# rom1504/clip-retrieval

Hardware: AMD Instinct MI355X
Metric: images/sec embedded (ViT-L/14 bs=256; each sample = image + caption through both towers) (higher is better)
Workload: dtype bf16

## Files before the change

clip-retrieval_amd/csrc/clip_kernels.h:

```cpp
#pragma once
#include <hip/hip_runtime.h>
#include <stdint.h>

namespace clipx {

typedef __bf16 bf16;

enum GemmEpilogue {
  EPI_BIAS_BF16 = 0,
  EPI_BIAS_QGELU_BF16 = 1,
  EPI_BIAS_GELU_BF16 = 2,
  EPI_BIAS_RESID_F32 = 3,
  EPI_TABLE_F32 = 4,
  EPI_RAW_F32 = 5,
  EPI_BIAS_RESID_H16 = 6,
  EPI_BIAS_F16 = 7
};

struct GemmArgs {
  const bf16* A;
  const bf16* W;
  const float* bias;
  void* out;
  const float* table;
  int T;
  int M, N, K;
  int epi;
  int variant;
  int n_cu;
  int row0;
  const float* rowscale;
  bf16* out16;
  float* splitk_ws;
  size_t splitk_ws_bytes;
  int tail_m0, tail_nb;
  int f16;
  float stats_eps;
  int* range_flag;
};

int gemm256_bulk_mtiles(int M, int N, int n_cu);
int gemm256_tail_blocks(int N, int K, int n_cu);

hipError_t launch_gemm(const GemmArgs& g, hipStream_t st);

hipError_t launch_layernorm(const float* x, const float* gamma, const float* beta, void* y, int out_kind, int M,
                            int d, float eps, hipStream_t st, bf16* y16 = nullptr);

hipError_t launch_rowstats(const void* x16, float* rstd, int M, int d, float eps, hipStream_t st, int f16 = 0, int* range_flag = nullptr,
                           int canonical = 0);

hipError_t launch_fold_layernorm(const float* W, const float* gamma, const float* beta, const float* bias, bf16* Wf, float* cf,
                                 int N, int K, hipStream_t st, int f16 = 0);
hipError_t launch_fill_f32(float* p, float v, int64_t n, hipStream_t st);

hipError_t launch_im2col(const void* pixels, int fmt, int B, int S, int P, int Kp, const float* mean,
                         const float* stdv, bf16* out, hipStream_t st);

hipError_t launch_attention(const bf16* qkv, bf16* out, int B, int T, int H, int dh, int causal, hipStream_t st, int q_blocks = 0,
                            const int* offs = nullptr, const int* lens = nullptr);

hipError_t launch_text_embed(const int32_t* ids, const float* tok_emb, const float* pos_emb, float* x, int B, int T,
                             int d, int vocab, hipStream_t st, void* x16 = nullptr, int x16_f16 = 0, const int* rowmap = nullptr,
                             int nrows = 0);

hipError_t launch_gather_pooled(const bf16* att, const void* x16, const int32_t* ids_or_null, bf16* attc, void* xc, int B, int T,
                                int d, hipStream_t st, const int* rows_or_null = nullptr);
hipError_t launch_tail(const void* x, const int32_t* ids_or_null, const float* gamma, const float* beta,
                       const bf16* proj, uint16_t* out_f16, float* out_f32_or_null, float* scratch, int B, int T, int d,
                       int E, float eps, hipStream_t st, int x_f16 = 0, int* range_flag = nullptr);

hipError_t launch_f32_to_bf16(const float* in, bf16* out, int64_t n, hipStream_t st);
hipError_t launch_pad_rows_bf16(const float* in, bf16* out, int rows, int k, int kp, hipStream_t st);

}
```

clip-retrieval_amd/csrc/clip_kernels.hip:

```cpp

#include <hip/hip_runtime.h>
#include <stdint.h>
#include <stdlib.h>
#include <math.h>
#include "clip_kernels.h"
#include "gemm_common.h"

namespace clipx {

constexpr int G_TM = 128, G_TN = 128, G_BK = 64;
constexpr int G_STAGE_BYTES = (G_TM + G_TN) * G_BK * 2;
constexpr int G_GROUP_M = 8;

template <int EPI, bool GLDS, bool DEEP = false, bool F16 = false>
__global__ __launch_bounds__(256, (DEEP && !CLIPX_MFMA16) ? 1 : 2) void gemm_bf16_kernel(const bf16* __restrict__ A, const bf16* __restrict__ W,
                                                          const float* __restrict__ bias, void* __restrict__ outp,
                                                          const float* __restrict__ table, int T, int M, int N,
                                                          int K, int row0, const float* __restrict__ rowscale,
                                                          bf16* __restrict__ out16, int kz) {
  extern __shared__ __attribute__((aligned(16))) unsigned char smem[];
  const int tid = threadIdx.x;
  const int lane = tid & 63, w = tid >> 6;
  const int wn = w & 1, wm = w >> 1;
  const int hb = lane >> 5, l31 = lane & 31;
// ... 375 lines not shown
}

static hipError_t launch_gemm128(const GemmArgs& g, hipStream_t st) {
  const bool small_off = (size_t)g.M * g.K * 2 < ((size_t)1 << 32) && (size_t)g.N * g.K * 2 < ((size_t)1 << 32);
  const int S = (g.variant == 1 && small_off) ? splitk_factor(g) : 1;
  if (S > 1) {
    switch (g.epi) {
      case EPI_BIAS_BF16: return launch_splitk_epi<EPI_BIAS_BF16>(g, S, st);
      case EPI_BIAS_F16: return launch_splitk_epi<EPI_BIAS_F16>(g, S, st);
      case EPI_BIAS_QGELU_BF16: return launch_splitk_epi<EPI_BIAS_QGELU_BF16>(g, S, st);
      case EPI_BIAS_GELU_BF16: return launch_splitk_epi<EPI_BIAS_GELU_BF16>(g, S, st);
      case EPI_BIAS_RESID_F32: return launch_splitk_epi<EPI_BIAS_RESID_F32>(g, S, st);
      case EPI_BIAS_RESID_H16: return launch_splitk_epi<EPI_BIAS_RESID_H16>(g, S, st);
      default: break;
    }
  }
  if (g.f16) {
    switch (g.epi) {
      case EPI_BIAS_BF16: return launch_gemm_epi<EPI_BIAS_BF16, true>(g, st);
      case EPI_BIAS_F16: return launch_gemm_epi<EPI_BIAS_F16, true>(g, st);
      case EPI_BIAS_QGELU_BF16: return launch_gemm_epi<EPI_BIAS_QGELU_BF16, true>(g, st);
      case EPI_BIAS_GELU_BF16: return launch_gemm_epi<EPI_BIAS_GELU_BF16, true>(g, st);
      default: return hipErrorInvalidValue;
    }
  }
  switch (g.epi) {
    case EPI_BIAS_BF16: return launch_gemm_epi<EPI_BIAS_BF16>(g, st);
    case EPI_BIAS_F16: return launch_gemm_epi<EPI_BIAS_F16>(g, st);
    case EPI_BIAS_QGELU_BF16: return launch_gemm_epi<EPI_BIAS_QGELU_BF16>(g, st);
    case EPI_BIAS_GELU_BF16: return launch_gemm_epi<EPI_BIAS_GELU_BF16>(g, st);
    case EPI_BIAS_RESID_F32: return launch_gemm_epi<EPI_BIAS_RESID_F32>(g, st);
    case EPI_BIAS_RESID_H16: return launch_gemm_epi<EPI_BIAS_RESID_H16>(g, st);
    case EPI_TABLE_F32: return launch_gemm_epi<EPI_TABLE_F32>(g, st);
    default: return hipErrorInvalidValue;
  }
}

int gemm256_bulk_mtiles(int M, int N, int n_cu) {
  const int mt = M / 256, nt = N / 256;
  if (mt <= 0 || nt <= 0) return 0;
  const int cu = (n_cu > 0 ? n_cu : 256) & ~7;
  int best = mt;
  double best_cost = 1e30;
  for (int peel = 0; peel <= 8 && peel < mt; ++peel) {
    const int bulk = mt - peel;
    const int rounds = (bulk * nt + cu - 1) / cu;
    const double rest = (double)(peel * 4 * nt) / (2.0 * cu);
    const double cost = rounds + (peel ? 0.25 * (rest > 1.0 ? rest : 1.0) / 0.6 : 0.0);
    if (cost < best_cost - 1e-9) { best_cost = cost; best = bulk; }
  }
  return best;
}

int gemm256_tail_blocks(int N, int K, int n_cu) {
  int grid = (n_cu > 0 ? n_cu : 256) & ~7;
  if (grid < 8) grid = 8;
  if (N % 32 || K % 128 || (size_t)32 * K * 2 >= ((size_t)1 << 31)) return 0;
  const int cb = N / 32;
  for (int nb = 1; nb <= 4; ++nb)
    if (cb % nb == 0 && 8 * (cb / nb) <= grid) return nb;
  return 0;
}

hipError_t launch_gemm(const GemmArgs& g0, hipStream_t st) {
  GemmArgs g = g0;
  if (g.M <= 0 || g.N % G_TN != 0 || g.K % G_BK != 0 || g.K <= 0) return hipErrorInvalidValue;
  const bool out16 = g.epi == EPI_BIAS_BF16 || g.epi == EPI_BIAS_QGELU_BF16 || g.epi == EPI_BIAS_GELU_BF16 || g.epi == EPI_BIAS_F16;
  if (out16 && !g.rowscale) return hipErrorInvalidValue;
  if (g.f16 && !out16) return hipErrorInvalidValue;
  if (g.stats_eps > 0.f) {
    if (!g.f16 || !out16) return hipErrorInvalidValue;
    int fused_rows = 0;
    if (g.variant == 6 && g.N % 256 == 0 && g.K % 128 == 0 && g.M >= 256) {
      const int bulk = gemm256_bulk_mtiles(g.M, g.N, g.n_cu);
      const int cu = (g.n_cu > 0 ? g.n_cu : 256);
      GemmArgs b = g;
      b.M = bulk * 256;
      if (bulk > 0 && (int64_t)bulk * (g.N / 256) >= cu / 2 && gemm256w4_fuses_stats(b)) fused_rows = b.M;
    }
    if (fused_rows < g.M) {
      hipError_t e = launch_rowstats(reinterpret_cast<const char*>(g.A) + (size_t)fused_rows * g.K * 2, const_cast<float*>(g.rowscale) + fused_rows,
                                     g.M - fused_rows, g.K, g.stats_eps, st, 1, g.range_flag, 1);
      if (e != hipSuccess) return e;
    }
    if (fused_rows == 0) g.stats_eps = 0.f;
  }
  if (g.variant >= 2 && g.N % 256 == 0 && g.K % 128 == 0 && g.M >= 256) {
    const int bulk = gemm256_bulk_mtiles(g.M, g.N, g.n_cu);
    const int cu = (g.n_cu > 0 ? g.n_cu : 256);
    if (bulk > 0 && (int64_t)bulk * (g.N / 256) >= cu / 2) {
      GemmArgs b = g;
      b.M = bulk * 256;
      b.tail_m0 = b.tail_nb = 0;
      if (g.M - b.M == 256 && (g.variant == 3 || g.variant == 6) && g.row0 == 0) {
        b.tail_nb = gemm256_tail_blocks(g.N, g.K, g.n_cu);
        b.tail_m0 = b.M;
      }
      const bool tail_inside = b.tail_nb > 0;
      hipError_t e = (g.variant == 6 && gemm256w4_supports(b)) ? launch_gemm256w4(b, g.n_cu, st) : launch_gemm256sp(b, g.n_cu, st);
      if (e != hipSuccess) return e;
      if (b.M == g.M || tail_inside) return hipSuccess;
      GemmArgs r = g;
      r.variant = 1;
      r.stats_eps = 0.f;
      r.splitk_ws = nullptr;
      r.A = g.A + (size_t)b.M * g.K;
      r.M = g.M - b.M;
      const size_t esz = (g.epi == EPI_BIAS_RESID_F32 || g.epi == EPI_TABLE_F32) ? 4 : 2;
      r.out = reinterpret_cast<char*>(g.out) + (size_t)b.M * g.N * esz;
      r.row0 = g.row0 + b.M;
      if (g.rowscale) r.rowscale = g.rowscale + b.M;
      if (g.out16) r.out16 = g.out16 + (size_t)b.M * g.N;
      return launch_gemm128(r, st);
    }
  }
  GemmArgs r = g;
  if (r.variant >= 2) r.variant = 1;
  r.stats_eps = 0.f;
  return launch_gemm128(r, st);
}

template <int NV, int OUT>
__global__ __launch_bounds__(256) void layernorm_kernel(const float* __restrict__ x, const float* __restrict__ gamma,
                                                       const float* __restrict__ beta, void* __restrict__ y, int M,
                                                       float eps, bf16* __restrict__ y16) {
  constexpr int d = NV * 256;
  const int lane = threadIdx.x & 63;
  const int row = blockIdx.x * 4 + (threadIdx.x >> 6);
  if (row >= M) return;
  const float4* xr = reinterpret_cast<const float4*>(x + (size_t)row * d);
  float4 v[NV];
  float s = 0.f;
#pragma unroll
  for (int e = 0; e < NV; ++e) {
    v[e] = xr[lane + 64 * e];
    s += (v[e].x + v[e].y) + (v[e].z + v[e].w);
  }
  for (int o = 32; o > 0; o >>= 1) s += __shfl_xor(s, o);
  const float mean = s * (1.f / d);
  float q = 0.f;
#pragma unroll
  for (int e = 0; e < NV; ++e) {
    const float a = v[e].x - mean, b = v[e].y - mean, c = v[e].z - mean, dd = v[e].w - mean;
    q += (a * a + b * b) + (c * c + dd * dd);
  }
  for (int o = 32; o > 0; o >>= 1) q += __shfl_xor(q, o);
  const float rstd = 1.f / sqrtf(q * (1.f / d) + eps);
#pragma unroll
  for (int e = 0; e < NV; ++e) {
    const int c4 = lane + 64 * e;
    const float4 g4 = reinterpret_cast<const float4*>(gamma)[c4];
    const float4 b4 = reinterpret_cast<const float4*>(beta)[c4];
    float4 o;
    o.x = (v[e].x - mean) * rstd * g4.x + b4.x;
    o.y = (v[e].y - mean) * rstd * g4.y + b4.y;
    o.z = (v[e].z - mean) * rstd * g4.z + b4.z;
    o.w = (v[e].w - mean) * rstd * g4.w + b4.w;
    if (OUT == 1) {
      bf16x4 ob;
      ob[0] = (bf16)o.x; ob[1] = (bf16)o.y; ob[2] = (bf16)o.z; ob[3] = (bf16)o.w;
      reinterpret_cast<bf16x4*>(reinterpret_cast<bf16*>(y) + (size_t)row * d)[c4] = ob;
    } else if (OUT == 2) {
      f16x4 oh;
      oh[0] = (_Float16)o.x; oh[1] = (_Float16)o.y; oh[2] = (_Float16)o.z; oh[3] = (_Float16)o.w;
      reinterpret_cast<f16x4*>(reinterpret_cast<_Float16*>(y) + (size_t)row * d)[c4] = oh;
    } else {
      reinterpret_cast<float4*>(reinterpret_cast<float*>(y) + (size_t)row * d)[c4] = o;
      if (y16) {
// ... 1265 lines not shown
```

clip-retrieval_amd/csrc/clipx_api.hip:

```cpp

#include <hip/hip_runtime.h>
#include <stdint.h>
#include <stdlib.h>
#include <string.h>
#include <algorithm>
#include <map>
#include <mutex>
#include <tuple>
#include <string>
#include <vector>

#include "../../include/clipx.h"
#include "clip_kernels.h"

using namespace clipx;

static thread_local std::string g_err;
static int fail(int code, const std::string& msg) {
  g_err = msg;
  return code;
}
#define HIPCHK(expr)                                                                      \
  do {                                                                                    \
    hipError_t _e = (expr);                                                               \
// ... 159 lines not shown
}

static int create_impl(clipx_handle* h, const float* blob, size_t blob_floats) {
  const clipx_model_desc& d = h->desc;
  const int g = d.image_size / d.patch_size;
  Tower& V = h->vis;
  Tower& X = h->txt;
  V.width = d.v_width; V.layers = d.v_layers; V.heads = d.v_heads; V.mlp = d.v_mlp; V.T = g * g + 1;
  X.width = d.t_width; X.layers = d.t_layers; X.heads = d.t_heads; X.mlp = d.t_mlp; X.T = d.ctx_len;
  h->PP3 = 3 * d.patch_size * d.patch_size;
  h->Kp = (h->PP3 + 63) / 64 * 64;
  const size_t E = d.embed_dim;

  HIPCHK(hipStreamCreateWithFlags(&h->stream, hipStreamNonBlocking));
  HIPCHK(hipStreamCreateWithFlags(&h->copy_stream, hipStreamNonBlocking));
  HIPCHK(hipMalloc((void**)&h->blob_dev, blob_floats * sizeof(float)));
  HIPCHK(hipMemcpy(h->blob_dev, blob, blob_floats * sizeof(float), hipMemcpyHostToDevice));

  int r;
  float* p = h->blob_dev;
  const float* conv32 = p; p += (size_t)V.width * h->PP3;
  const float* cls = p; p += V.width;
  const float* vpos = p; p += (size_t)V.T * V.width;
  h->ln_pre_w = p; p += V.width;
  h->ln_pre_b = p; p += V.width;
  if ((r = dev_alloc(h, (void**)&h->conv_w, (size_t)V.width * h->Kp * sizeof(bf16)))) return r;
  HIPCHK(launch_pad_rows_bf16(conv32, h->conv_w, V.width, h->PP3, h->Kp, h->stream));
  if ((r = dev_alloc(h, (void**)&h->clspos, (size_t)V.T * V.width * sizeof(float)))) return r;
  HIPCHK(hipMemcpyAsync(h->clspos, vpos, (size_t)V.T * V.width * sizeof(float), hipMemcpyDeviceToDevice, h->stream));
  {
    const size_t off_cls = (size_t)(cls - h->blob_dev), off_pos = (size_t)(vpos - h->blob_dev);
    std::vector<float> row0(V.width);
    for (int i = 0; i < V.width; ++i) row0[i] = blob[off_cls + i] + blob[off_pos + i];
    HIPCHK(hipStreamSynchronize(h->stream));
    HIPCHK(hipMemcpy(h->clspos, row0.data(), V.width * sizeof(float), hipMemcpyHostToDevice));
  }
  if ((r = carve_layers(h, V, p))) return r;
  V.lnf_w = p; p += V.width;
  V.lnf_b = p; p += V.width;
  const float* vproj32 = p; p += E * V.width;
  if ((r = dev_alloc(h, (void**)&V.proj, E * V.width * sizeof(bf16)))) return r;
  HIPCHK(launch_f32_to_bf16(vproj32, V.proj, (int64_t)(E * V.width), h->stream));
  h->tok_emb = p; p += (size_t)d.vocab * X.width;
  h->txt_pos = p; p += (size_t)X.T * X.width;
  if ((r = carve_layers(h, X, p))) return r;
  X.lnf_w = p; p += X.width;
  X.lnf_b = p; p += X.width;
  const float* tproj32 = p; p += E * X.width;
  if ((r = dev_alloc(h, (void**)&X.proj, E * X.width * sizeof(bf16)))) return r;
  HIPCHK(launch_f32_to_bf16(tproj32, X.proj, (int64_t)(E * X.width), h->stream));
  if ((size_t)(p - h->blob_dev) != blob_floats) return fail(CLIPX_E_ARG, "internal: blob carve does not match clipx_blob_floats");

  const size_t Bm = h->max_batch;
  const size_t rowsV = Bm * V.T, rowsX = Bm * X.T;
  const size_t nx = std::max(rowsV * V.width, rowsX * X.width);
  const size_t nqkv = std::max(rowsV * 3 * V.width, rowsX * 3 * X.width);
  const size_t nh = std::max(rowsV * V.mlp, rowsX * X.mlp);
  if ((r = dev_alloc(h, (void**)&h->x, rowsV * V.width * sizeof(float)))) return r;
  if ((r = dev_alloc(h, (void**)&h->xn, nx * sizeof(bf16)))) return r;
  if ((r = dev_alloc(h, (void**)&h->rstd, std::max(rowsV, rowsX) * sizeof(float)))) return r;
  if ((r = dev_alloc(h, (void**)&h->qkv, nqkv * sizeof(bf16)))) return r;
  if ((r = dev_alloc(h, (void**)&h->att, nx * sizeof(bf16)))) return r;
  if ((r = dev_alloc(h, (void**)&h->hbuf, nh * sizeof(bf16)))) return r;
  if ((r = dev_alloc(h, (void**)&h->patches, rowsV * h->Kp * sizeof(bf16)))) return r;
  h->splitk_ws_bytes = (size_t)32 << 20;
  if ((r = dev_alloc(h, (void**)&h->splitk_ws, h->splitk_ws_bytes))) return r;

  h->in_slot_bytes = std::max((size_t)Bm * 3 * d.image_size * d.image_size * sizeof(float), (size_t)Bm * d.ctx_len * sizeof(int32_t));
  h->out_slot_bytes = Bm * E * sizeof(uint16_t);
  for (int s = 0; s < clipx_handle::NSLOT; ++s) {
    HIPCHK(hipHostMalloc(&h->pin_in[s], h->in_slot_bytes, hipHostMallocDefault));
    HIPCHK(hipHostMalloc(&h->pin_out[s], h->out_slot_bytes * 3, hipHostMallocDefault));
    if ((r = dev_alloc(h, &h->dev_in[s], h->in_slot_bytes))) return r;
    if ((r = dev_alloc(h, (void**)&h->dev_out[s], h->out_slot_bytes))) return r;
    if ((r = dev_alloc(h, (void**)&h->dev_out32[s], h->out_slot_bytes * 2))) return r;
    HIPCHK(hipEventCreateWithFlags(&h->ev_copied[s], hipEventDisableTiming));
    HIPCHK(hipEventCreateWithFlags(&h->ev_done[s], hipEventDisableTiming));
  }
  HIPCHK(hipEventCreateWithFlags(&h->ev_ws, hipEventDisableTiming));
  if ((r = dev_alloc(h, (void**)&h->range_flags, (clipx_handle::NSLOT + 1) * sizeof(int)))) return r;
  HIPCHK(hipMemsetAsync(h->range_flags, 0, (clipx_handle::NSLOT + 1) * sizeof(int), h->stream));
  HIPCHK(hipHostMalloc((void**)&h->range_host, (clipx_handle::NSLOT + 1) * sizeof(int), hipHostMallocDefault));
  memset(h->range_host, 0, (clipx_handle::NSLOT + 1) * sizeof(int));
  h->cur_flag = h->range_flags + clipx_handle::NSLOT;
  {
    const size_t rg_ints = (size_t)Bm * (X.T + 3);
    for (int i = 0; i < clipx_handle::RG_SLOTS; ++i) {
      HIPCHK(hipHostMalloc((void**)&h->rg_host[i], rg_ints * sizeof(int), hipHostMallocDefault));
      if ((r = dev_alloc(h, (void**)&h->rg_dev[i], rg_ints * sizeof(int)))) return r;
      HIPCHK(hipEventCreateWithFlags(&h->rg_ev[i], hipEventDisableTiming));
    }
    HIPCHK(hipHostMalloc((void**)&h->rg_ids_host, (size_t)Bm * X.T * sizeof(int32_t), hipHostMallocDefault));
  }
  HIPCHK(hipStreamSynchronize(h->stream));
  return 0;
}

extern "C" int clipx_create(const clipx_model_desc* desc, const float* blob, size_t blob_floats, int device,
                            clipx_handle** out) {
  if (!desc || !blob || !out) return fail(CLIPX_E_ARG, "null argument");
  *out = nullptr;
  int r = check_desc(desc);
  if (r) return r;
  if (blob_floats != clipx_blob_floats(desc)) return fail(CLIPX_E_ARG, "weight blob has the wrong number of floats for this model description");
  int ndev = 0;
  HIPCHK(hipGetDeviceCount(&ndev));
  if (device < 0 || device >= ndev) return fail(CLIPX_E_ARG, "no such HIP device");
  HIPCHK(hipSetDevice(device));
  hipDeviceProp_t prop;
  HIPCHK(hipGetDeviceProperties(&prop, device));
  if (std::string(prop.gcnArchName).find("gfx950") == std::string::npos)
    return fail(CLIPX_E_UNSUPPORTED, std::string("kernels are built for gfx950 only, device is ") + prop.gcnArchName);
  clipx_handle* h = new clipx_handle();
  h->desc = *desc;
  h->device = device;
  const char* mb = getenv("CLIPX_MAX_BATCH");
  if (mb && atoi(mb) > 0) h->max_batch = atoi(mb);
  const char* hc = getenv("CLIPX_HOST_CHUNK");
  if (hc && atoi(hc) > 0) h->host_chunk = atoi(hc);
  h->host_chunk = std::min(h->host_chunk, h->max_batch);
  const char* gv = getenv("CLIPX_GEMM_VARIANT");
  if (gv) h->gemm_variant = std::min(6, std::max(0, atoi(gv)));
  const char* lf = getenv("CLIPX_LN_FUSED");
  if (lf) h->ln_fused = lf[0] == '1';
  const char* rgt = getenv("CLIPX_RAGGED_TEXT");
  if (rgt && rgt[0] == '0') h->ragged_text = false;
  const char* fl = getenv("CLIPX_FULL_LAST_BLOCK");
  if (fl && atoi(fl) > 0) h->pool_last_block = false;
  h->n_cu = prop.multiProcessorCount > 0 ? prop.multiProcessorCount : 256;
  r = create_impl(h, blob, blob_floats);
  if (r) {
    std::string keep = g_err;
    clipx_destroy(h);
    g_err = keep;
    return r;
  }
  *out = h;
  return CLIPX_OK;
}
// ... 22 lines not shown
    if (h->rg_ev[i]) (void)hipEventDestroy(h->rg_ev[i]);
  }
  if (h->rg_ids_host) (void)hipHostFree(h->rg_ids_host);
  if (h->range_host) (void)hipHostFree(h->range_host);
  if (h->stream) (void)hipStreamDestroy(h->stream);
  if (h->copy_stream) (void)hipStreamDestroy(h->copy_stream);
  delete h;
}

extern "C" int clipx_set_option(clipx_handle* h, int option, int value) {
  if (!h) return fail(CLIPX_E_ARG, "handle is null");
  std::lock_guard<std::mutex> lk(h->mu);
  switch (option) {
    case CLIPX_OPT_RAGGED_TEXT: h->ragged_text = value != 0; return CLIPX_OK;
    case CLIPX_OPT_POOL_LAST_BLOCK: h->pool_last_block = value != 0; return CLIPX_OK;
    default: return fail(CLIPX_E_ARG, "unknown option");
  }
}
extern "C" int clipx_get_option(const clipx_handle* h, int option) {
  if (!h) return -1;
  switch (option) {
    case CLIPX_OPT_RAGGED_TEXT: return h->ragged_text ? 1 : 0;
    case CLIPX_OPT_POOL_LAST_BLOCK: return h->pool_last_block ? 1 : 0;
    default: return -1;
  }
}
extern "C" int clipx_max_batch(const clipx_handle* h) { return h ? h->max_batch : 0; }
extern "C" int clipx_graphs_cached(const clipx_handle* h) { return h ? (int)h->graphs.size() : 0; }
extern "C" int clipx_embed_dim(const clipx_handle* h) { return h ? h->desc.embed_dim : 0; }

struct ProfScope {
  clipx_handle* h;
  hipStream_t st;
  hipEvent_t a = nullptr, b = nullptr;
  int kind;
  double flops;
  ProfScope(clipx_handle* h_, hipStream_t st_, int kind_, double flops_) : h(h_), st(st_), kind(kind_), flops(flops_) {
    if (h->prof & (1 << kind)) {
      (void)hipEventCreate(&a);
      (void)hipEventCreate(&b);
      (void)hipEventRecord(a, st);
    }
  }
  ~ProfScope() {
    if (a && b) {
      (void)hipEventRecord(b, st);
      h->prof_events.push_back({a, b, kind, flops});
    }
  }
};

static int run_gemm(clipx_handle* h, hipStream_t st, const bf16* A, const bf16* W, const float* bias, void* out,
                    const float* table, int T, int M, int N, int K, int epi, const float* rowscale = nullptr, bool f16 = false,
                    float stats_eps = 0.f) {
  GemmArgs g{};
  g.A = A; g.W = W; g.bias = bias; g.out = out; g.table = table; g.T = T;
  g.M = M; g.N = N; g.K = K; g.epi = epi; g.variant = h->gemm_variant; g.n_cu = h->n_cu; g.row0 = 0;
  g.rowscale = rowscale; g.out16 = nullptr; g.f16 = f16 ? 1 : 0;
  g.stats_eps = stats_eps; g.range_flag = stats_eps > 0.f ? h->cur_flag : nullptr;
  if (h->single_query) { g.splitk_ws = h->splitk_ws; g.splitk_ws_bytes = h->splitk_ws_bytes; }
  ProfScope ps(h, st, 0, 2.0 * M * (double)N * K);
  HIPCHK(launch_gemm(g, st));
  return 0;
}

static const void* pooled_rows(const clipx_handle* h, int B, int width) {
  return reinterpret_cast<const char*>(h->x) + (((size_t)B * width * sizeof(bf16) + 255) & ~(size_t)255);
}

struct Ragged {
  int M;
  const int* offs;
  const int* lens;
  const int* rowmap;
  const int* poolrows;
  double att_flops;
};

static int run_layers(clipx_handle* h, hipStream_t st, const Tower& t, int B, int causal, const int32_t* ids, bool* pooled,
                      const Ragged* rg = nullptr) {
  const int M = rg ? rg->M : B * t.T, w = t.width;
  const float eps = h->desc.ln_eps;
  const int act = h->desc.act == CLIPX_ACT_QUICK_GELU ? EPI_BIAS_QGELU_BF16 : EPI_BIAS_GELU_BF16;
  for (int l = 0; l < t.layers; ++l) {
    const LayerW& L = t.L[l];
    int r;
    if (!h->ln_fused) { ProfScope ps(h, st, 2, 0); HIPCHK(launch_rowstats(h->xn, h->rstd, M, w, eps, st, 1, h->cur_flag)); }
    if ((r = run_gemm(h, st, h->xn, L.qkv_w, L.qkv_c, h->qkv, nullptr, 1, M, 3 * w, w, EPI_BIAS_F16, h->rstd, true, h->ln_fused ? eps : 0.f))) return r;
    const bool pool_here = l == t.layers - 1 && h->pool_last_block && t.T > 1;
    const int q_blocks = pool_here && !ids ? 1 : 0;
    const double att_rows = q_blocks ? std::min(32, t.T) : t.T;
    { ProfScope ps(h, st, 1, rg ? rg->att_flops * t.heads * (w / t.heads) : 4.0 * B * t.heads * att_rows * t.T * (w / t.heads));
      HIPCHK(launch_attention(h->qkv, h->att, B, t.T, t.heads, w / t.heads, causal, st, q_blocks, rg ? rg->offs : nullptr, rg ? rg->lens : nullptr)); }
    if (pool_here) {
      bf16* attc = reinterpret_cast<bf16*>(h->x);
      void* xc = reinterpret_cast<char*>(h->x) + (((size_t)B * w * sizeof(bf16) + 255) & ~(size_t)255);
      { ProfScope ps(h, st, 3, 0); HIPCHK(launch_gather_pooled(h->att, h->xn, ids, attc, xc, B, t.T, w, st, rg ? rg->poolrows : nullptr)); }
      if ((r = run_gemm(h, st, attc, L.out_w, L.out_b, xc, nullptr, 1, B, w, w, EPI_BIAS_RESID_H16))) return r;
      if (!h->ln_fused) { ProfScope ps(h, st, 2, 0); HIPCHK(launch_rowstats(xc, h->rstd, B, w, eps, st, 1, h->cur_flag)); }
      if ((r = run_gemm(h, st, reinterpret_cast<const bf16*>(xc), L.fc1_w, L.fc1_c, h->hbuf, nullptr, 1, B, t.mlp, w, act, h->rstd, true, h->ln_fused ? eps : 0.f))) return r;
      if ((r = run_gemm(h, st, h->hbuf, L.fc2_w, L.fc2_b, xc, nullptr, 1, B, w, t.mlp, EPI_BIAS_RESID_H16))) return r;
      *pooled = true;
      return 0;
    }
    if ((r = run_gemm(h, st, h->att, L.out_w, L.out_b, h->xn, nullptr, 1, M, w, w, EPI_BIAS_RESID_H16))) return r;
    if (!h->ln_fused) { ProfScope ps(h, st, 2, 0); HIPCHK(launch_rowstats(h->xn, h->rstd, M, w, eps, st, 1, h->cur_flag)); }
    if ((r = run_gemm(h, st, h->xn, L.fc1_w, L.fc1_c, h->hbuf, nullptr, 1, M, t.mlp, w, act, h->rstd, true, h->ln_fused ? eps : 0.f))) return r;
    if ((r = run_gemm(h, st, h->hbuf, L.fc2_w, L.fc2_b, h->xn, nullptr, 1, M, w, t.mlp, EPI_BIAS_RESID_H16))) return r;
  }
  *pooled = false;
  return 0;
}

constexpr int GRAPH_MAX_B = 8;
constexpr size_t GRAPH_MAX = 64;

template <class F>
static int run_graphed(clipx_handle* h, hipStream_t st, const clipx_handle::GraphKey& key, int B, F&& body) {
  if (!h->graphs_on || h->prof || B > GRAPH_MAX_B) return body();
  auto it = h->graphs.find(key);
  if (it != h->graphs.end()) {
    HIPCHK(hipGraphLaunch(it->second, st));
    return 0;
  }
  if (h->graphs.size() >= GRAPH_MAX) return body();
  if (h->graph_seen.size() > 4 * GRAPH_MAX) h->graph_seen.clear();
  if (++h->graph_seen[key] < 2) return body();
  if (hipStreamBeginCapture(st, hipStreamCaptureModeRelaxed) != hipSuccess) {
    (void)hipGetLastError();
    h->graphs_on = false;
    return body();
  }
  const int r = body();
  hipGraph_t g = nullptr;
  const hipError_t e = hipStreamEndCapture(st, &g);
  hipGraphExec_t ex = nullptr;
  if (r == 0 && e == hipSuccess && g && hipGraphInstantiate(&ex, g, nullptr, nullptr, 0) == hipSuccess) {
    (void)hipGraphDestroy(g);
    h->graphs[key] = ex;
    HIPCHK(hipGraphLaunch(ex, st));
    return 0;
  }
  if (g) (void)hipGraphDestroy(g);
  (void)hipGetLastError();
  h->graphs_on = false;
  return body();
}

static int vision_chunk_body(clipx_handle* h, hipStream_t st, const void* pix_dev, int B, int fmt, uint16_t* out_f16,
                             float* out_f32);
static int text_chunk_body(clipx_handle* h, hipStream_t st, const int32_t* ids_dev, int B, uint16_t* out_f16, float* out_f32);
static bool stream_is_capturing(hipStream_t st);

static int vision_chunk(clipx_handle* h, hipStream_t st, const void* pix_dev, int B, int fmt, uint16_t* out_f16,
                        float* out_f32) {
  return run_graphed(h, st, clipx_handle::GraphKey(h->single_query ? 16 : 0, B, fmt, pix_dev, out_f16, out_f32, st), B,
                     [&]() { return vision_chunk_body(h, st, pix_dev, B, fmt, out_f16, out_f32); });
}

static int text_chunk(clipx_handle* h, hipStream_t st, const int32_t* ids_dev, int B, uint16_t* out_f16, float* out_f32) {
  return run_graphed(h, st, clipx_handle::GraphKey(h->single_query ? 17 : 1, B, 0, ids_dev, out_f16, out_f32, st), B,
                     [&]() { return text_chunk_body(h, st, ids_dev, B, out_f16, out_f32); });
}

static int vision_chunk_body(clipx_handle* h, hipStream_t st, const void* pix_dev, int B, int fmt, uint16_t* out_f16,
                             float* out_f32) {
  const clipx_model_desc& d = h->desc;
  const Tower& V = h->vis;
  const int M = B * V.T;
  { ProfScope ps(h, st, 3, 0); HIPCHK(launch_im2col(pix_dev, fmt, B, d.image_size, d.patch_size, h->Kp, d.pix_mean, d.pix_std, h->patches, st)); }
  int r = run_gemm(h, st, h->patches, h->conv_w, nullptr, h->x, h->clspos, V.T, M, V.width, h->Kp, EPI_TABLE_F32);
  if (r) return r;
  { ProfScope ps(h, st, 2, 0); HIPCHK(launch_layernorm(h->x, h->ln_pre_w, h->ln_pre_b, h->xn, 2, M, V.width, d.ln_eps, st)); }
  bool pooled = false;
  if ((r = run_layers(h, st, V, B, 0, nullptr, &pooled))) return r;
  const void* xf = pooled ? pooled_rows(h, B, V.width) : h->xn;
  { ProfScope ps(h, st, 3, 0); HIPCHK(launch_tail(xf, nullptr, V.lnf_w, V.lnf_b, V.proj, out_f16, out_f32, reinterpret_cast<float*>(h->qkv), B, pooled ? 1 : V.T, V.width, d.embed_dim, d.ln_eps, st, 1, h->cur_flag)); }
  return 0;
}

static int ragged_prepare(clipx_handle* h, hipStream_t st, const int32_t* ids_host, int B, Ragged* rg) {
  const int T = h->txt.T;
  const int s = h->rg_next;
  h->rg_next = (s + 1) % clipx_handle::RG_SLOTS;
  if (h->rg_used[s]) HIPCHK(hipEventSynchronize(h->rg_ev[s]));
  int* host = h->rg_host[s];
  int* offs = host, *lens = host + B, *pool = host + 2 * B, *rowmap = host + 3 * B;
  int M = 0;
  double f = 0.0;
  for (int b = 0; b < B; ++b) {
    const int32_t* row = ids_host + (size_t)b * T;
    int best = 0, bv = row[0];
    for (int t = 1; t < T; ++t)
      if (row[t] > bv) { bv = row[t]; best = t; }
    const int len = best + 1;
    offs[b] = M;
    lens[b] = len;
    pool[b] = M + best;
    for (int t = 0; t < len; ++t) rowmap[M + t] = b * T + t;
    M += len;
    f += 4.0 * (double)len * len;
  }
  int* dev = h->rg_dev[s];
  HIPCHK(hipMemcpyAsync(dev, host, ((size_t)3 * B + M) * sizeof(int), hipMemcpyHostToDevice, st));
  HIPCHK(hipEventRecord(h->rg_ev[s], st));
  h->rg_used[s] = true;
  rg->M = M;
  rg->offs = dev;
  rg->lens = dev + B;
  rg->poolrows = dev + 2 * B;
  rg->rowmap = dev + 3 * B;
  rg->att_flops = f;
  return 0;
}

static int text_chunk_body(clipx_handle* h, hipStream_t st, const int32_t* ids_dev, int B, uint16_t* out_f16, float* out_f32) {
  const clipx_model_desc& d = h->desc;
  const Tower& X = h->txt;
  Ragged rgv{};
  const Ragged* rg = nullptr;
  bool ragged = h->ragged_text && h->pool_last_block && B > GRAPH_MAX_B && X.T <= 128 && X.width / X.heads == 64;
  if (ragged && stream_is_capturing(st)) ragged = false;
  if (ragged) {
    const int32_t* ids_host = h->text_ids_host;
    if (!ids_host) {
      HIPCHK(hipMemcpyAsync(h->rg_ids_host, ids_dev, (size_t)B * X.T * sizeof(int32_t), hipMemcpyDeviceToHost, st));
      HIPCHK(hipStreamSynchronize(st));
      ids_host = h->rg_ids_host;
    }
    int rr = ragged_prepare(h, st, ids_host, B, &rgv);
    if (rr) return rr;
    rg = &rgv;
  }
  { ProfScope ps(h, st, 3, 0); HIPCHK(launch_text_embed(ids_dev, h->tok_emb, h->txt_pos, nullptr, B, X.T, X.width, d.vocab, st, h->xn, 1, rg ? rg->rowmap : nullptr, rg ? rg->M : 0)); }
  bool pooled = false;
  int r = run_layers(h, st, X, B, 1, ids_dev, &pooled, rg);
  if (r) return r;
  const void* xf = pooled ? pooled_rows(h, B, X.width) : h->xn;
  { ProfScope ps(h, st, 3, 0); HIPCHK(launch_tail(xf, pooled ? nullptr : ids_dev, X.lnf_w, X.lnf_b, X.proj, out_f16, out_f32, reinterpret_cast<float*>(h->qkv), B, pooled ? 1 : X.T, X.width, d.embed_dim, d.ln_eps, st, 1, h->cur_flag)); }
  return 0;
}

static bool stream_is_capturing(hipStream_t st) {
  hipStreamCaptureStatus cs = hipStreamCaptureStatusNone;
  if (hipStreamIsCapturing(st, &cs) != hipSuccess) { (void)hipGetLastError(); return false; }
  return cs != hipStreamCaptureStatusNone;
}
static int ws_acquire(clipx_handle* h, hipStream_t st) {
  if (h->ev_ws_valid && !stream_is_capturing(st)) HIPCHK(hipStreamWaitEvent(st, h->ev_ws, 0));
  return 0;
}
static int ws_release(clipx_handle* h, hipStream_t st) {
  if (stream_is_capturing(st)) return 0;
  HIPCHK(hipEventRecord(h->ev_ws, st));
  h->ev_ws_valid = true;
  return 0;
}

static size_t pix_bytes_per_image(const clipx_model_desc& d, int fmt) {
  const size_t px = (size_t)3 * d.image_size * d.image_size;
  return fmt == CLIPX_PIX_F32_NCHW ? px * sizeof(float) : px;
}

extern "C" int clipx_encode_image_device(clipx_handle* h, const void* pixels_dev, int B, int pix_fmt, uint16_t* out_f16_dev,
                                         float* out_f32_or_null, void* stream) {
  if (!h || !pixels_dev || !out_f16_dev || B < 0) return fail(CLIPX_E_ARG, "bad encode_image arguments");
  if (pix_fmt != CLIPX_PIX_F32_NCHW && pix_fmt != CLIPX_PIX_U8_NHWC) return fail(CLIPX_E_ARG, "unknown pixel format");
  std::lock_guard<std::mutex> lk(h->mu);
  HIPCHK(hipSetDevice(h->device));
  hipStream_t st = stream ? (hipStream_t)stream : h->stream;
  const size_t ib = pix_bytes_per_image(h->desc, pix_fmt), E = h->desc.embed_dim;
  h->single_query = B == 1;
  h->cur_flag = h->range_flags + clipx_handle::NSLOT;
  if (ws_acquire(h, st)) return CLIPX_E_HIP;
  for (int o = 0; o < B; o += h->max_batch) {
    const int nb = std::min(h->max_batch, B - o);
    int r = vision_chunk(h, st, (const char*)pixels_dev + (size_t)o * ib, nb, pix_fmt, out_f16_dev + (size_t)o * E,
                         out_f32_or_null ? out_f32_or_null + (size_t)o * E : nullptr);
    if (r) return r;
  }
  if (ws_release(h, st)) return CLIPX_E_HIP;
  return CLIPX_OK;
}

static int encode_text_device_impl(clipx_handle* h, const int32_t* ids_dev, const int32_t* ids_host_or_null, int B, uint16_t* out_f16_dev,
                                   float* out_f32_or_null, void* stream);

// ... 342 lines not shown
```

clip-retrieval_amd/csrc/gemm_common.h:

```cpp
#pragma once
#include <hip/hip_runtime.h>
#include <stdint.h>
#include "clip_kernels.h"

namespace clipx {

typedef __bf16 bf16x8 __attribute__((ext_vector_type(8)));
typedef __bf16 bf16x4 __attribute__((ext_vector_type(4)));
typedef float f32x16 __attribute__((ext_vector_type(16)));
typedef float f32x4 __attribute__((ext_vector_type(4)));
typedef _Float16 f16x8 __attribute__((ext_vector_type(8)));
typedef _Float16 f16x4 __attribute__((ext_vector_type(4)));
typedef int frag_t __attribute__((ext_vector_type(4)));

template <bool F16>
__device__ __forceinline__ f32x16 mfma_32x32x16(frag_t a, frag_t b, f32x16 c) {
  if constexpr (F16) return __builtin_amdgcn_mfma_f32_32x32x16_f16(__builtin_bit_cast(f16x8, a), __builtin_bit_cast(f16x8, b), c, 0, 0, 0);
  else return __builtin_amdgcn_mfma_f32_32x32x16_bf16(__builtin_bit_cast(bf16x8, a), __builtin_bit_cast(bf16x8, b), c, 0, 0, 0);
}
#ifndef CLIPX_MFMA16
#define CLIPX_MFMA16 1
#endif

template <bool F16>
// ... 47 lines not shown
  if (EPI == EPI_RAW_F32) {
    *reinterpret_cast<float4*>(reinterpret_cast<float*>(outp) + (size_t)m * N + n) = v;
    return;
  }
  if (EPI != EPI_TABLE_F32) {
    const float4 b4 = *reinterpret_cast<const float4*>(bias + n);
    if (OUT_BF16) {
      const float r = rowscale[m];
      v.x = __builtin_fmaf(v.x, r, b4.x); v.y = __builtin_fmaf(v.y, r, b4.y);
      v.z = __builtin_fmaf(v.z, r, b4.z); v.w = __builtin_fmaf(v.w, r, b4.w);
    } else {
      v.x += b4.x; v.y += b4.y; v.z += b4.z; v.w += b4.w;
    }
  }
  if (EPI == EPI_BIAS_QGELU_BF16) { v.x = quick_gelu(v.x); v.y = quick_gelu(v.y); v.z = quick_gelu(v.z); v.w = quick_gelu(v.w); }
  if (EPI == EPI_BIAS_GELU_BF16) { v.x = gelu_erf(v.x); v.y = gelu_erf(v.y); v.z = gelu_erf(v.z); v.w = gelu_erf(v.w); }
  if (EPI == EPI_BIAS_F16) {
    asm volatile("" : "+v"(v.x), "+v"(v.y), "+v"(v.z), "+v"(v.w));
    f16x4 o;
    o[0] = (_Float16)v.x; o[1] = (_Float16)v.y; o[2] = (_Float16)v.z; o[3] = (_Float16)v.w;
    *reinterpret_cast<f16x4*>(reinterpret_cast<_Float16*>(outp) + (size_t)m * N + n) = o;
  } else if (OUT_BF16) {
    bf16x4 o;
    o[0] = (bf16)v.x; o[1] = (bf16)v.y; o[2] = (bf16)v.z; o[3] = (bf16)v.w;
    *reinterpret_cast<bf16x4*>(reinterpret_cast<bf16*>(outp) + (size_t)m * N + n) = o;
  } else if (EPI == EPI_BIAS_RESID_F32) {
    float4* p = reinterpret_cast<float4*>(reinterpret_cast<float*>(outp) + (size_t)m * N + n);
    float4 o = *p;
    o.x += v.x; o.y += v.y; o.z += v.z; o.w += v.w;
    *p = o;
    if (out16) {
      bf16x4 h;
      h[0] = (bf16)o.x; h[1] = (bf16)o.y; h[2] = (bf16)o.z; h[3] = (bf16)o.w;
      *reinterpret_cast<bf16x4*>(out16 + (size_t)m * N + n) = h;
    }
  } else if (EPI == EPI_BIAS_RESID_H16) {
    f16x4* p = reinterpret_cast<f16x4*>(reinterpret_cast<_Float16*>(outp) + (size_t)m * N + n);
    const f16x4 x4 = *p;
    f16x4 h;
    h[0] = (_Float16)((float)x4[0] + v.x); h[1] = (_Float16)((float)x4[1] + v.y);
    h[2] = (_Float16)((float)x4[2] + v.z); h[3] = (_Float16)((float)x4[3] + v.w);
    *p = h;
  } else {
    const float4 t4 = *reinterpret_cast<const float4*>(table + (size_t)((m + row0) % T) * N + n);
    v.x += t4.x; v.y += t4.y; v.z += t4.z; v.w += t4.w;
    *reinterpret_cast<float4*>(reinterpret_cast<float*>(outp) + (size_t)m * N + n) = v;
  }
}

hipError_t launch_gemm256sp(const GemmArgs& g, int n_cu, hipStream_t st);
bool gemm256w4_supports(const GemmArgs& g);
bool gemm256w4_fuses_stats(const GemmArgs& g);
hipError_t launch_gemm256w4(const GemmArgs& g, int n_cu, hipStream_t st);

}
```

Measured before the change: 5966.

## Pad ragged text rows to whole 256-row tiles and add strip GEMM path

The ragged text tower's token count is padded up to a multiple of 256 using dummy copies of the longest sample, so the text GEMMs can take the 256x256 tile path instead of splitting off a remainder handled by the 128-tile kernel. A new strip GEMM kernel, reusing the existing 256-row tail routine, handles M==256 GEMMs for the MLP and residual epilogues. The aim is to avoid the slower remainder kernels and the poor occupancy of small-M GEMMs. In exchange, padded rows do extra GEMM and attention work, and the ragged metadata layout and buffer sizes change.

```diff
diff --git a/clip-retrieval_amd/csrc/clip_kernels.h b/clip-retrieval_amd/csrc/clip_kernels.h
--- a/clip-retrieval_amd/csrc/clip_kernels.h
+++ b/clip-retrieval_amd/csrc/clip_kernels.h
@@ -40,6 +40,7 @@
 };
 
 int gemm256_bulk_mtiles(int M, int N, int n_cu);
+bool gemm256_takes_whole_tiles(int M, int N, int K, int variant, int n_cu);
 int gemm256_tail_blocks(int N, int K, int n_cu);
 
 hipError_t launch_gemm(const GemmArgs& g, hipStream_t st);
diff --git a/clip-retrieval_amd/csrc/clip_kernels.hip b/clip-retrieval_amd/csrc/clip_kernels.hip
--- a/clip-retrieval_amd/csrc/clip_kernels.hip
+++ b/clip-retrieval_amd/csrc/clip_kernels.hip
@@ -451,6 +451,13 @@
   return best;
 }
 
+bool gemm256_takes_whole_tiles(int M, int N, int K, int variant, int n_cu) {
+  if (variant < 2 || N % 256 != 0 || K % 128 != 0 || M < 256) return false;
+  const int bulk = gemm256_bulk_mtiles(M, N, n_cu);
+  const int cu = (n_cu > 0 ? n_cu : 256);
+  return bulk > 0 && (int64_t)bulk * (N / 256) >= cu / 2;
+}
+
 int gemm256_tail_blocks(int N, int K, int n_cu) {
   int grid = (n_cu > 0 ? n_cu : 256) & ~7;
   if (grid < 8) grid = 8;
@@ -470,12 +477,10 @@
   if (g.stats_eps > 0.f) {
     if (!g.f16 || !out16) return hipErrorInvalidValue;
     int fused_rows = 0;
-    if (g.variant == 6 && g.N % 256 == 0 && g.K % 128 == 0 && g.M >= 256) {
-      const int bulk = gemm256_bulk_mtiles(g.M, g.N, g.n_cu);
-      const int cu = (g.n_cu > 0 ? g.n_cu : 256);
+    if (g.variant == 6 && gemm256_takes_whole_tiles(g.M, g.N, g.K, g.variant, g.n_cu)) {
       GemmArgs b = g;
-      b.M = bulk * 256;
-      if (bulk > 0 && (int64_t)bulk * (g.N / 256) >= cu / 2 && gemm256w4_fuses_stats(b)) fused_rows = b.M;
+      b.M = gemm256_bulk_mtiles(g.M, g.N, g.n_cu) * 256;
+      if (gemm256w4_fuses_stats(b)) fused_rows = b.M;
     }
     if (fused_rows < g.M) {
       hipError_t e = launch_rowstats(reinterpret_cast<const char*>(g.A) + (size_t)fused_rows * g.K * 2, const_cast<float*>(g.rowscale) + fused_rows,
@@ -484,35 +489,33 @@
     }
     if (fused_rows == 0) g.stats_eps = 0.f;
   }
-  if (g.variant >= 2 && g.N % 256 == 0 && g.K % 128 == 0 && g.M >= 256) {
+  if (gemm256_takes_whole_tiles(g.M, g.N, g.K, g.variant, g.n_cu)) {
     const int bulk = gemm256_bulk_mtiles(g.M, g.N, g.n_cu);
-    const int cu = (g.n_cu > 0 ? g.n_cu : 256);
-    if (bulk > 0 && (int64_t)bulk * (g.N / 256) >= cu / 2) {
-      GemmArgs b = g;
-      b.M = bulk * 256;
-      b.tail_m0 = b.tail_nb = 0;
-      if (g.M - b.M == 256 && (g.variant == 3 || g.variant == 6) && g.row0 == 0) {
-        b.tail_nb = gemm256_tail_blocks(g.N, g.K, g.n_cu);
-        b.tail_m0 = b.M;
-      }
-      const bool tail_inside = b.tail_nb > 0;
-      hipError_t e = (g.variant == 6 && gemm256w4_supports(b)) ? launch_gemm256w4(b, g.n_cu, st) : launch_gemm256sp(b, g.n_cu, st);
-      if (e != hipSuccess) return e;
-      if (b.M == g.M || tail_inside) return hipSuccess;
-      GemmArgs r = g;
-      r.variant = 1;
-      r.stats_eps = 0.f;
-      r.splitk_ws = nullptr;
-      r.A = g.A + (size_t)b.M * g.K;
-      r.M = g.M - b.M;
-      const size_t esz = (g.epi == EPI_BIAS_RESID_F32 || g.epi == EPI_TABLE_F32) ? 4 : 2;
-      r.out = reinterpret_cast<char*>(g.out) + (size_t)b.M * g.N * esz;
-      r.row0 = g.row0 + b.M;
-      if (g.rowscale) r.rowscale = g.rowscale + b.M;
-      if (g.out16) r.out16 = g.out16 + (size_t)b.M * g.N;
-      return launch_gemm128(r, st);
-    }
-  }
+    GemmArgs b = g;
+    b.M = bulk * 256;
+    b.tail_m0 = b.tail_nb = 0;
+    if (g.M - b.M == 256 && (g.variant == 3 || g.variant == 6) && g.row0 == 0) {
+      b.tail_nb = gemm256_tail_blocks(g.N, g.K, g.n_cu);
+      b.tail_m0 = b.M;
+    }
+    const bool tail_inside = b.tail_nb > 0;
+    hipError_t e = (g.variant == 6 && gemm256w4_supports(b)) ? launch_gemm256w4(b, g.n_cu, st) : launch_gemm256sp(b, g.n_cu, st);
+    if (e != hipSuccess) return e;
+    if (b.M == g.M || tail_inside) return hipSuccess;
+    GemmArgs r = g;
+    r.variant = 1;
+    r.stats_eps = 0.f;
+    r.splitk_ws = nullptr;
+    r.A = g.A + (size_t)b.M * g.K;
+    r.M = g.M - b.M;
+    const size_t esz = (g.epi == EPI_BIAS_RESID_F32 || g.epi == EPI_TABLE_F32) ? 4 : 2;
+    r.out = reinterpret_cast<char*>(g.out) + (size_t)b.M * g.N * esz;
+    r.row0 = g.row0 + b.M;
+    if (g.rowscale) r.rowscale = g.rowscale + b.M;
+    if (g.out16) r.out16 = g.out16 + (size_t)b.M * g.N;
+    return launch_gemm128(r, st);
+  }
+  if (g.variant >= 2 && !g.splitk_ws && gemm_strip_supports(g)) return launch_gemm_strip(g, st);
   GemmArgs r = g;
   if (r.variant >= 2) r.variant = 1;
   r.stats_eps = 0.f;
diff --git a/clip-retrieval_amd/csrc/clipx_api.hip b/clip-retrieval_amd/csrc/clipx_api.hip
--- a/clip-retrieval_amd/csrc/clipx_api.hip
+++ b/clip-retrieval_amd/csrc/clipx_api.hip
@@ -235,7 +235,7 @@
   if ((size_t)(p - h->blob_dev) != blob_floats) return fail(CLIPX_E_ARG, "internal: blob carve does not match clipx_blob_floats");
 
   const size_t Bm = h->max_batch;
-  const size_t rowsV = Bm * V.T, rowsX = Bm * X.T;
+  const size_t rowsV = Bm * V.T, rowsX = (Bm * X.T + 255) / 256 * 256;
   const size_t nx = std::max(rowsV * V.width, rowsX * X.width);
   const size_t nqkv = std::max(rowsV * 3 * V.width, rowsX * 3 * X.width);
   const size_t nh = std::max(rowsV * V.mlp, rowsX * X.mlp);
@@ -267,7 +267,7 @@
   memset(h->range_host, 0, (clipx_handle::NSLOT + 1) * sizeof(int));
   h->cur_flag = h->range_flags + clipx_handle::NSLOT;
   {
-    const size_t rg_ints = (size_t)Bm * (X.T + 3);
+    const size_t rg_ints = (size_t)Bm + 2 * ((size_t)Bm + 255) + rowsX;
     for (int i = 0; i < clipx_handle::RG_SLOTS; ++i) {
       HIPCHK(hipHostMalloc((void**)&h->rg_host[i], rg_ints * sizeof(int), hipHostMallocDefault));
       if ((r = dev_alloc(h, (void**)&h->rg_dev[i], rg_ints * sizeof(int)))) return r;
@@ -396,14 +396,14 @@
 
 static int run_gemm(clipx_handle* h, hipStream_t st, const bf16* A, const bf16* W, const float* bias, void* out,
                     const float* table, int T, int M, int N, int K, int epi, const float* rowscale = nullptr, bool f16 = false,
-                    float stats_eps = 0.f) {
+                    float stats_eps = 0.f, int flop_rows = 0) {
   GemmArgs g{};
   g.A = A; g.W = W; g.bias = bias; g.out = out; g.table = table; g.T = T;
   g.M = M; g.N = N; g.K = K; g.epi = epi; g.variant = h->gemm_variant; g.n_cu = h->n_cu; g.row0 = 0;
   g.rowscale = rowscale; g.out16 = nullptr; g.f16 = f16 ? 1 : 0;
   g.stats_eps = stats_eps; g.range_flag = stats_eps > 0.f ? h->cur_flag : nullptr;
   if (h->single_query) { g.splitk_ws = h->splitk_ws; g.splitk_ws_bytes = h->splitk_ws_bytes; }
-  ProfScope ps(h, st, 0, 2.0 * M * (double)N * K);
+  ProfScope ps(h, st, 0, 2.0 * (flop_rows > 0 ? flop_rows : M) * (double)N * K);
   HIPCHK(launch_gemm(g, st));
   return 0;
 }
@@ -414,6 +414,8 @@
 
 struct Ragged {
   int M;
+  int Mp;
+  int samples;
   const int* offs;
   const int* lens;
   const int* rowmap;
@@ -423,19 +425,20 @@
 
 static int run_layers(clipx_handle* h, hipStream_t st, const Tower& t, int B, int causal, const int32_t* ids, bool* pooled,
                       const Ragged* rg = nullptr) {
-  const int M = rg ? rg->M : B * t.T, w = t.width;
+  const int M = rg ? rg->Mp : B * t.T, w = t.width;
+  const int Mf = rg ? rg->M : M;
   const float eps = h->desc.ln_eps;
   const int act = h->desc.act == CLIPX_ACT_QUICK_GELU ? EPI_BIAS_QGELU_BF16 : EPI_BIAS_GELU_BF16;
   for (int l = 0; l < t.layers; ++l) {
     const LayerW& L = t.L[l];
     int r;
     if (!h->ln_fused) { ProfScope ps(h, st, 2, 0); HIPCHK(launch_rowstats(h->xn, h->rstd, M, w, eps, st, 1, h->cur_flag)); }
-    if ((r = run_gemm(h, st, h->xn, L.qkv_w, L.qkv_c, h->qkv, nullptr, 1, M, 3 * w, w, EPI_BIAS_F16, h->rstd, true, h->ln_fused ? eps : 0.f))) return r;
+    if ((r = run_gemm(h, st, h->xn, L.qkv_w, L.qkv_c, h->qkv, nullptr, 1, M, 3 * w, w, EPI_BIAS_F16, h->rstd, true, h->ln_fused ? eps : 0.f, Mf))) return r;
     const bool pool_here = l == t.layers - 1 && h->pool_last_block && t.T > 1;
     const int q_blocks = pool_here && !ids ? 1 : 0;
     const double att_rows = q_blocks ? std::min(32, t.T) : t.T;
     { ProfScope ps(h, st, 1, rg ? rg->att_flops * t.heads * (w / t.heads) : 4.0 * B * t.heads * att_rows * t.T * (w / t.heads));
-      HIPCHK(launch_attention(h->qkv, h->att, B, t.T, t.heads, w / t.heads, causal, st, q_blocks, rg ? rg->offs : nullptr, rg ? rg->lens : nullptr)); }
+      HIPCHK(launch_attention(h->qkv, h->att, rg ? rg->samples : B, t.T, t.heads, w / t.heads, causal, st, q_blocks, rg ? rg->offs : nullptr, rg ? rg->lens : nullptr)); }
     if (pool_here) {
       bf16* attc = reinterpret_cast<bf16*>(h->x);
       void* xc = reinterpret_cast<char*>(h->x) + (((size_t)B * w * sizeof(bf16) + 255) & ~(size_t)255);
@@ -447,10 +450,10 @@
       *pooled = true;
       return 0;
     }
-    if ((r = run_gemm(h, st, h->att, L.out_w, L.out_b, h->xn, nullptr, 1, M, w, w, EPI_BIAS_RESID_H16))) return r;
+    if ((r = run_gemm(h, st, h->att, L.out_w, L.out_b, h->xn, nullptr, 1, M, w, w, EPI_BIAS_RESID_H16, nullptr, false, 0.f, Mf))) return r;
     if (!h->ln_fused) { ProfScope ps(h, st, 2, 0); HIPCHK(launch_rowstats(h->xn, h->rstd, M, w, eps, st, 1, h->cur_flag)); }
-    if ((r = run_gemm(h, st, h->xn, L.fc1_w, L.fc1_c, h->hbuf, nullptr, 1, M, t.mlp, w, act, h->rstd, true, h->ln_fused ? eps : 0.f))) return r;
-    if ((r = run_gemm(h, st, h->hbuf, L.fc2_w, L.fc2_b, h->xn, nullptr, 1, M, w, t.mlp, EPI_BIAS_RESID_H16))) return r;
+    if ((r = run_gemm(h, st, h->xn, L.fc1_w, L.fc1_c, h->hbuf, nullptr, 1, M, t.mlp, w, act, h->rstd, true, h->ln_fused ? eps : 0.f, Mf))) return r;
+    if ((r = run_gemm(h, st, h->hbuf, L.fc2_w, L.fc2_b, h->xn, nullptr, 1, M, w, t.mlp, EPI_BIAS_RESID_H16, nullptr, false, 0.f, Mf))) return r;
   }
   *pooled = false;
   return 0;
@@ -524,36 +527,51 @@
 }
 
 static int ragged_prepare(clipx_handle* h, hipStream_t st, const int32_t* ids_host, int B, Ragged* rg) {
-  const int T = h->txt.T;
+  const Tower& X = h->txt;
+  const int T = X.T;
   const int s = h->rg_next;
   h->rg_next = (s + 1) % clipx_handle::RG_SLOTS;
   if (h->rg_used[s]) HIPCHK(hipEventSynchronize(h->rg_ev[s]));
   int* host = h->rg_host[s];
-  int* offs = host, *lens = host + B, *pool = host + 2 * B, *rowmap = host + 3 * B;
-  int M = 0;
+  int* pool = host;
+  int M = 0, longest = 0;
   double f = 0.0;
   for (int b = 0; b < B; ++b) {
     const int32_t* row = ids_host + (size_t)b * T;
     int best = 0, bv = row[0];
     for (int t = 1; t < T; ++t)
       if (row[t] > bv) { bv = row[t]; best = t; }
-    const int len = best + 1;
-    offs[b] = M;
+    pool[b] = best;
+    if (best > pool[longest]) longest = b;
+    M += best + 1;
+    f += 4.0 * (double)(best + 1) * (best + 1);
+  }
+  const int Mr = (M + 255) / 256 * 256;
+  const int Mp = gemm256_takes_whole_tiles(Mr, 3 * X.width, X.width, h->gemm_variant, h->n_cu) ? Mr : M;
+  const int lmax = pool[longest] + 1;
+  const int P = (Mp - M + lmax - 1) / lmax;
+  int* offs = host + B, *lens = offs + B + P, *rowmap = lens + B + P;
+  int m = 0;
+  for (int b = 0; b < B + P; ++b) {
+    const int src = b < B ? b : longest;
+    const int len = b < B ? pool[b] + 1 : std::min(lmax, Mp - m);
+    offs[b] = m;
     lens[b] = len;
-    pool[b] = M + best;
-    for (int t = 0; t < len; ++t) rowmap[M + t] = b * T + t;
-    M += len;
-    f += 4.0 * (double)len * len;
+    if (b < B) pool[b] = m + len - 1;
+    for (int t = 0; t < len; ++t) rowmap[m + t] = src * T + t;
+    m += len;
   }
   int* dev = h->rg_dev[s];
-  HIPCHK(hipMemcpyAsync(dev, host, ((size_t)3 * B + M) * sizeof(int), hipMemcpyHostToDevice, st));
+  HIPCHK(hipMemcpyAsync(dev, host, ((size_t)B + 2 * (size_t)(B + P) + Mp) * sizeof(int), hipMemcpyHostToDevice, st));
   HIPCHK(hipEventRecord(h->rg_ev[s], st));
   h->rg_used[s] = true;
   rg->M = M;
-  rg->offs = dev;
-  rg->lens = dev + B;
-  rg->poolrows = dev + 2 * B;
-  rg->rowmap = dev + 3 * B;
+  rg->Mp = Mp;
+  rg->samples = B + P;
+  rg->poolrows = dev;
+  rg->offs = dev + B;
+  rg->lens = dev + 2 * B + P;
+  rg->rowmap = dev + 3 * B + 2 * P;
   rg->att_flops = f;
   return 0;
 }
@@ -576,7 +594,7 @@
     if (rr) return rr;
     rg = &rgv;
   }
-  { ProfScope ps(h, st, 3, 0); HIPCHK(launch_text_embed(ids_dev, h->tok_emb, h->txt_pos, nullptr, B, X.T, X.width, d.vocab, st, h->xn, 1, rg ? rg->rowmap : nullptr, rg ? rg->M : 0)); }
+  { ProfScope ps(h, st, 3, 0); HIPCHK(launch_text_embed(ids_dev, h->tok_emb, h->txt_pos, nullptr, B, X.T, X.width, d.vocab, st, h->xn, 1, rg ? rg->rowmap : nullptr, rg ? rg->Mp : 0)); }
   bool pooled = false;
   int r = run_layers(h, st, X, B, 1, ids_dev, &pooled, rg);
   if (r) return r;
diff --git a/clip-retrieval_amd/csrc/gemm_common.h b/clip-retrieval_amd/csrc/gemm_common.h
--- a/clip-retrieval_amd/csrc/gemm_common.h
+++ b/clip-retrieval_amd/csrc/gemm_common.h
@@ -123,5 +123,7 @@
 bool gemm256w4_supports(const GemmArgs& g);
 bool gemm256w4_fuses_stats(const GemmArgs& g);
 hipError_t launch_gemm256w4(const GemmArgs& g, int n_cu, hipStream_t st);
+bool gemm_strip_supports(const GemmArgs& g);
+hipError_t launch_gemm_strip(const GemmArgs& g, hipStream_t st);
 
 }
diff --git a/clip-retrieval_amd/csrc/gemm_strip.hip b/clip-retrieval_amd/csrc/gemm_strip.hip
--- /dev/null
+++ b/clip-retrieval_amd/csrc/gemm_strip.hip
@@ -0,0 +1,57 @@
+
+#include <hip/hip_runtime.h>
+#include <stdint.h>
+#include "gemm_common.h"
+#include "gemm256_tail.h"
+
+namespace clipx {
+
+constexpr int STRIP_LDS = 131072;
+
+template <int EPI, bool F16, int NB>
+__global__ __launch_bounds__(256, 1) void gemm_strip_kernel(const bf16* __restrict__ A, const bf16* __restrict__ W,
+                                                           const float* __restrict__ bias, void* __restrict__ outp, int N, int K,
+                                                           const float* __restrict__ rowscale) {
+  extern __shared__ __attribute__((aligned(16))) unsigned char smem[];
+  const int lane = threadIdx.x & 63;
+  const int w = __builtin_amdgcn_readfirstlane(threadIdx.x >> 6);
+  const unsigned lds_base = __builtin_amdgcn_readfirstlane((unsigned)(uintptr_t)(__attribute__((address_space(3))) unsigned char*)smem);
+  gemm256_tail<EPI, F16, NB, 4>(A, W, bias, outp, nullptr, 1, N, K, rowscale, nullptr, 0, smem, lds_base, w, lane);
+}
+
+template <int EPI, bool F16, int NB>
+static hipError_t launch_strip_nb(const GemmArgs& g, hipStream_t st) {
+  auto kern = gemm_strip_kernel<EPI, F16, NB>;
+  hipError_t e = hipFuncSetAttribute(reinterpret_cast<const void*>(kern), hipFuncAttributeMaxDynamicSharedMemorySize, STRIP_LDS);
+  if (e != hipSuccess) return e;
+  const int strips = 8 * ((g.N / 32) / NB);
+  hipLaunchKernelGGL(kern, dim3(strips), dim3(256), STRIP_LDS, st, g.A, g.W, g.bias, g.out, g.N, g.K, g.rowscale);
+  return hipGetLastError();
+}
+
+template <int EPI, bool F16>
+static hipError_t launch_strip_epi(const GemmArgs& g, int nb, hipStream_t st) {
+  switch (nb) {
+    case 1: return launch_strip_nb<EPI, F16, 1>(g, st);
+    case 2: return launch_strip_nb<EPI, F16, 2>(g, st);
+    case 3: return launch_strip_nb<EPI, F16, 3>(g, st);
+    case 4: return launch_strip_nb<EPI, F16, 4>(g, st);
+    default: return hipErrorInvalidValue;
+  }
+}
+
+bool gemm_strip_supports(const GemmArgs& g) {
+  if (g.M != 256 || g.row0 != 0 || g.K <= 0 || gemm256_tail_blocks(g.N, g.K, g.n_cu) <= 0) return false;
+  if (g.f16) return (g.epi == EPI_BIAS_QGELU_BF16 || g.epi == EPI_BIAS_GELU_BF16) && g.rowscale != nullptr;
+  return g.epi == EPI_BIAS_RESID_H16;
+}
+
+hipError_t launch_gemm_strip(const GemmArgs& g, hipStream_t st) {
+  if (!gemm_strip_supports(g)) return hipErrorInvalidValue;
+  const int nb = gemm256_tail_blocks(g.N, g.K, g.n_cu);
+  if (!g.f16) return launch_strip_epi<EPI_BIAS_RESID_H16, false>(g, nb, st);
+  if (g.epi == EPI_BIAS_QGELU_BF16) return launch_strip_epi<EPI_BIAS_QGELU_BF16, true>(g, nb, st);
+  return launch_strip_epi<EPI_BIAS_GELU_BF16, true>(g, nb, st);
+}
+
+}
```

Result: no change. 6014, median of 6 (+0.8%).
